# e4s2022/e4s

Hardware: AMD Instinct MI355X
Metric: 1024^2 face-swap images/sec (higher is better)
Workload: dtype f32 operands as hi+lo bf16, 3 bf16 MFMAs per product, f32 accumulate (bf16x3) on the 3x3 convs whose launch fills the chip; exact f32 elsewhere; 1 GPU; E4S-core face swap at 1024^2 (2x Net3 encoder @256^2, style swap, 12 LocalMLPs, mask-guided StyleGAN2 generator K=13), BASELINE.json configs[3] shard: 8 swaps per GPU per step; per_gpu_batch=8, global_batch=8, out_size=1024, hip_graph=True, precision=as bf16x3 where the launch fills the chip (this batch), else exact fp32, parallelism=image-parallel x1

## Files before the change

e4s_amd/csrc/common.h:

```cpp
#pragma once
#include <hip/hip_runtime.h>
#include <stdint.h>
#include <atomic>
#include "e4s_hip.h"

typedef float f32x4 __attribute__((ext_vector_type(4)));
typedef float f32x16 __attribute__((ext_vector_type(16)));

#define E4S_CHECK_LAUNCH()                         \
    do {                                           \
        hipError_t e__ = hipGetLastError();        \
        if (e__ != hipSuccess) return (int)e__;    \
    } while (0)

static inline hipStream_t as_stream(void* s) { return reinterpret_cast<hipStream_t>(s); }

__device__ __forceinline__ float wave_sum(float v) {
#pragma unroll
    for (int o = 32; o > 0; o >>= 1) v += __shfl_xor(v, o, 64);
    return v;
}

template <int N, int CNT, int O>
__device__ __forceinline__ void packed_wave_sum_step(float (&v)[N], const int lane) {
// ... 26 lines not shown
               : __int_as_float(__builtin_amdgcn_mov_dpp(__float_as_int(v), 0x4E, 0xF, 0xF, true));
}

__device__ __forceinline__ void quad_transpose4(float& a0, float& a1, float& a2, float& a3, const int lane) {
    const bool odd = lane & 1, hi = lane & 2;
    const float r01 = e4s_dpp_f32(odd ? a0 : a1, 0xB1), r23 = e4s_dpp_f32(odd ? a2 : a3, 0xB1);
    if (odd) { a0 = r01; a2 = r23; } else { a1 = r01; a3 = r23; }
    const float ra = e4s_dpp_f32(hi ? a0 : a2, 0x4E), rb = e4s_dpp_f32(hi ? a1 : a3, 0x4E);
    if (hi) { a0 = ra; a1 = rb; } else { a2 = ra; a3 = rb; }
}

__device__ __forceinline__ int xcd_remap(int bid, int nblk) {
    const int q = nblk >> 3, r = nblk & 7;
    const int xcd = bid & 7, slot = bid >> 3;
    const int base = (xcd < r) ? xcd * (q + 1) : r * (q + 1) + (xcd - r) * q;
    return base + slot;
}

static inline int e4s_ensure_dyn_smem(const void* fn, int bytes, std::atomic<uint64_t>& mask) {
    int dev = 0;
    hipError_t e = hipGetDevice(&dev);
    if (e != hipSuccess) return (int)e;
    const uint64_t bit = 1ull << (dev & 63);
    if (mask.load(std::memory_order_acquire) & bit) return 0;
    e = hipFuncSetAttribute(fn, hipFuncAttributeMaxDynamicSharedMemorySize, bytes);
    if (e != hipSuccess) return (int)e;
    mask.fetch_or(bit, std::memory_order_release);
    return 0;
}

int e4s_splitk_epilogue(const e4s_conv_params& p, int ksplit, hipStream_t st);

static inline int cdiv(int64_t a, int64_t b) { return (int)((a + b - 1) / b); }
```

e4s_amd/csrc/conv_bf16x3.hip:

```cpp
#include "common.h"
#include <stdlib.h>

namespace {

typedef __bf16 bf16x8 __attribute__((ext_vector_type(8)));
typedef float f32x8 __attribute__((ext_vector_type(8)));

constexpr int KC = 32;
constexpr int ROWB = 144;
constexpr int LO = 64;
constexpr int TW = 16, HALO_W = TW + 2;
constexpr int PBM = 256, PTH = 16, PHALO = (PTH + 2) * HALO_W;
constexpr int PNTHR = 512;

template <int BN_, int WM_, int WN_, int TPS_, int KCH_ = 32>
struct PCfg {
    static constexpr int BN = BN_, WM = WM_, WN = WN_, TPS = TPS_, KCH = KCH_;
    static constexpr int TM = PBM / (WM * 32), TN = BN / (WN * 32);
    static constexpr int ROWB = KCH == 32 ? 144 : 80;
    static constexpr int LO = KCH * 2;
    static constexpr int QG = KCH / 8;
    static constexpr int KSTEPS = KCH / 16;
    static constexpr int ITEMS = PHALO * QG;
    static constexpr int A_BYTES = PHALO * ROWB;
// ... 1115 lines not shown
    static_assert(SMEM <= 160 * 1024, "LDS budget");
    static std::atomic<uint64_t> smem_set{0};
    if (int e = e4s_ensure_dyn_smem(reinterpret_cast<const void*>(kern), SMEM, smem_set)) return e;
    const int ngemm = SHUF ? 4 * p.Cout : p.Cout;
    const int ntn = ngemm / C::BN;
    const int tx_n = (p.Wa + TW - 1) / TW, per_img = ((p.Ha + PTH - 1) / PTH) * tx_n;
    int ksplit, cper;
    plain_split(p, ngemm / C::BN, ksplit, cper);
    cper *= 32 / C::KCH;
    if (ksplit > 1 && !p.splitk_ws) return (int)hipErrorInvalidValue;
    const int64_t ntiles = (int64_t)p.B * per_img * ntn * ksplit;
    if (ntiles <= 0) return 0;
    if (ntiles >= (1ll << 31)) return (int)hipErrorInvalidValue;
    const int grid = (int)(ntiles < num_cus() ? ntiles : num_cus());
    hipLaunchKernelGGL(kern, dim3((unsigned)grid), dim3(PNTHR), SMEM, st, p, ntn, tx_n, per_img, (int)ntiles, ksplit, cper);
    E4S_CHECK_LAUNCH();
    if (ksplit > 1) {
        const int ycs = p.y_cstride ? p.y_cstride : p.Cout;
        const int64_t npix = (int64_t)p.B * p.Ho * p.Wo;
        const int64_t n4 = npix * (p.Cout / 4);
        hipLaunchKernelGGL(splitk_epilogue_kernel, dim3((unsigned)((n4 + 255) / 256)), dim3(256), 0, st, p, ksplit, ycs,
                           (int64_t)p.Ho * p.Wo, n4);
        E4S_CHECK_LAUNCH();
    }
    return 0;
}

template <typename C, bool SHUF>
int launch_xf(const e4s_conv_params& p, hipStream_t st) {
    if (p.in_stats) return SHUF ? (int)hipErrorInvalidValue : launch<C, 2, false>(p, st);
    return p.in_scale ? launch<C, 1, SHUF>(p, st) : launch<C, 0, SHUF>(p, st);
}

}

int e4s_launch_region_select(const e4s_conv_params& p, const int* only_flagged, hipStream_t st) {
    return launch_region(p, only_flagged, st);
}
void e4s_region_split_policy(const e4s_conv_params& p, int& ksplit, int& cper) { region_split(p, ksplit, cper); }

extern "C" int e4s_conv_bf16x3_f32(const e4s_conv_params* pp, void* stream) {
    const e4s_conv_params& p = *pp;
    const bool up = (p.ncls == 4);
    if (p.istride == 2 || p.ntaps == 1) {
        if (p.Cin % KC || (p.Cout % BN && p.Cout != 64) || (p.ntaps != 9 && p.ntaps != 1) || p.ncls != 1 || p.ostride != 1 || p.tiles ||
            p.labels || p.in_scale || p.out_scale || p.in_stats || p.noise || p.Ho != p.Ha || p.Wo != p.Wa ||
            p.Hi >= 32767 || p.Wi >= 32767 || (p.Ha - 1) * p.istride >= p.Hi || (p.Wa - 1) * p.istride >= p.Wi ||
            p.tap_shift < 0 || p.tap_shift > 1 ||
            (p.stats_ws && (p.act != 0 || (p.Ha * p.Wa) % BM || p.stats_slots != (p.Ha * p.Wa) / BM)))
            return (int)hipErrorInvalidValue;
        return launch_gather(p, as_stream(stream));
    }
    if (p.Cin % KC || p.Cout % 32 || p.ntaps != 9 || (p.ncls != 1 && !up) || p.istride != 1 ||
        p.ostride != (up ? 2 : 1) || p.tiles || p.noise_per_channel || p.Ha != p.Hi || p.Wa != p.Wi ||
        p.Ho != p.Hi * p.ostride || p.Wo != p.Wi * p.ostride || (p.in_stats && p.in_scale))
        return (int)hipErrorInvalidValue;
    if (p.stats_ws && (p.labels || up || p.act != 0 || p.noise || p.out_scale ||
                       p.stats_slots != ((p.Ha + PTH - 1) / PTH) * ((p.Wa + TW - 1) / TW)))
        return (int)hipErrorInvalidValue;
    hipStream_t st = as_stream(stream);
    if (p.labels) {
        if (p.y_cstride || !p.in_scale || p.in_stats || p.act == 2 || p.Cout % BN || p.groups_per_batch < 1 || p.groups_per_batch > MAXR)
            return (int)hipErrorInvalidValue;
        return launch_region(p, nullptr, st);
    }
#ifdef E4S_ABLATIONS
    static const int abl = [] { const char* e = getenv("E4S_BF16X3_ABL"); return e ? atoi(e) : 0; }();
    if (abl && !up && p.Cout % 128 == 0 && !p.in_stats && !p.in_scale) {
        switch (abl) {
            case 1: return launch<CfgL, 0, false, 1>(p, st);
            case 2: return launch<CfgL, 0, false, 2>(p, st);
            case 3: return launch<CfgL, 0, false, 3>(p, st);
            case 4: return launch<CfgL, 0, false, 4>(p, st);
            case 5: return launch<CfgL, 0, false, 5>(p, st);
            default: break;
        }
    }
#endif
    if (up) {
        if ((4 * p.Cout) % 128) return (int)hipErrorInvalidValue;
        return launch_xf<CfgL, true>(p, st);
    }
// ... 5 lines not shown
    if (p.Cout % 64 == 0) return launch_xf<CfgM, false>(p, st);
    return launch_xf<CfgS, false>(p, st);
}

int e4s_splitk_epilogue(const e4s_conv_params& p, int ksplit, hipStream_t st) {
    if (!p.splitk_ws || ksplit < 2 || p.Cout % 4) return (int)hipErrorInvalidValue;
    e4s_conv_params q = p;
    q.out_scale = nullptr;
    const int ycs = p.y_cstride ? p.y_cstride : p.Cout;
    const int64_t n4 = (int64_t)p.B * p.Ho * p.Wo * (p.Cout / 4);
    hipLaunchKernelGGL(splitk_epilogue_kernel, dim3((unsigned)((n4 + 255) / 256)), dim3(256), 0, st, q, ksplit, ycs,
                       (int64_t)p.Ho * p.Wo, n4);
    E4S_CHECK_LAUNCH();
    return 0;
}

extern "C" int64_t e4s_conv_bf16x3_ws_floats(const e4s_conv_params* pp) {
    const e4s_conv_params& p = *pp;
    if (p.istride != 1 || p.ntaps != 9 || p.Cin % KC) return 0;
    if (p.labels) {
        int ksplit, cper;
        region_split(p, ksplit, cper);
        return ksplit > 1 ? (int64_t)ksplit * p.B * p.Ho * p.Wo * p.Cout : 0;
    }
    const bool up = (p.ncls == 4);
    const int ngemm = up ? 4 * p.Cout : p.Cout;
    const int bn = (up || p.Cout % 128 == 0) ? 128 : (p.Cout % 64 == 0 ? 64 : 32);
    int ksplit, cper;
    plain_split(p, ngemm / bn, ksplit, cper);
    if (ksplit <= 1) return 0;
    return (int64_t)ksplit * p.B * p.Ho * p.Wo * (p.y_cstride ? p.y_cstride : p.Cout);
}

extern "C" int e4s_split_bf16x2_f32(const float* w, void* out, int64_t rows, int cin, void* stream) {
    if (cin % 32) return (int)hipErrorInvalidValue;
    const int64_t n8 = rows * (cin / 8);
    if (n8 <= 0) return 0;
    hipLaunchKernelGGL(split_bf16x2_kernel, dim3(cdiv(n8, 256)), dim3(256), 0, as_stream(stream), w,
                       reinterpret_cast<unsigned short*>(out), n8, cin);
    E4S_CHECK_LAUNCH();
    return 0;
}
```

e4s_amd/csrc/ops.hip:

```cpp
#include "common.h"

namespace {

__device__ __forceinline__ float bias_act_one(float x, float ref, int code, float alpha, float scale) {
    float y;
    switch (code) {
        case 12: case 32: y = 0.f; break;
        case 30: y = (x > 0.f) ? x : x * alpha; break;
        case 31: y = (ref > 0.f) ? x : x * alpha; break;
        default: y = x; break;
    }
    return y * scale;
}

__global__ void fused_bias_act_v4(const f32x4* __restrict__ x, const float* __restrict__ b,
                                  const f32x4* __restrict__ ref, f32x4* __restrict__ y, int64_t n4,
                                  int step_b, int size_b, int code, float alpha, float scale) {
    const int64_t stride = (int64_t)gridDim.x * blockDim.x;
    for (int64_t i = (int64_t)blockIdx.x * blockDim.x + threadIdx.x; i < n4; i += stride) {
        f32x4 v = x[i];
        if (b) {
            const float bv = b[((i * 4) / step_b) % size_b];
            v += bv;
        }
// ... 57 lines not shown
    for (int t = threadIdx.x; t < kh * kw; t += blockDim.x) {
        const int ky = t / kw, kx = t - ky * kw;
        sk[t] = k[(kh - 1 - ky) * kw + (kw - 1 - kx)];
    }
    const int mid_y0 = oy0 * down_y - pad_y0, mid_x0 = ox0 * down_x - pad_x0;
    const int in_y0 = floordiv(mid_y0 + up_y - 1, up_y), in_x0 = floordiv(mid_x0 + up_x - 1, up_x);
    for (int t = threadIdx.x; t < tin_h * tin_w; t += blockDim.x) {
        const int ry = t / tin_w, rx = t - ry * tin_w;
        const int iy = in_y0 + ry, ix = in_x0 + rx;
        float v = 0.f;
        if (iy >= 0 && ix >= 0 && iy < in_h && ix < in_w)
            v = x[(((int64_t)mj * in_h + iy) * in_w + ix) * minor + mi];
        sx[t] = v;
    }
    __syncthreads();
    for (int t = threadIdx.x; t < TOH * TOW; t += blockDim.x) {
        const int ry = t / TOW, rx = t - ry * TOW;
        const int oy = oy0 + ry, ox = ox0 + rx;
        if (oy >= out_h || ox >= out_w) continue;
        const int my = oy * down_y - pad_y0, mx = ox * down_x - pad_x0;
        const int iy_first = floordiv(my + up_y - 1, up_y), ix_first = floordiv(mx + up_x - 1, up_x);
        float acc = 0.f;
        for (int iy = iy_first, jy = iy_first * up_y - my; jy < kh; ++iy, jy += up_y) {
            const float* row = sx + (iy - in_y0) * tin_w;
            for (int ix = ix_first, jx = ix_first * up_x - mx; jx < kw; ++ix, jx += up_x)
                acc += row[ix - in_x0] * sk[jy * kw + jx];
        }
        y[(((int64_t)mj * out_h + oy) * out_w + ox) * minor + mi] = acc;
    }
}

}

extern "C" int e4s_abi_version(void) { return 16; }
extern "C" const char* e4s_build_arch(void) { return "gfx950"; }

extern "C" int e4s_fused_bias_act_f32(const float* x, const float* b, const float* ref, float* y, int64_t n,
                                      int step_b, int size_b, int act, int grad, float alpha, float scale,
                                      void* stream) {
    if (n <= 0) return 0;
    const int code = act * 10 + grad;
    if (code == 31 && !ref) return (int)hipErrorInvalidValue;
    if (b && (step_b <= 0 || size_b <= 0)) return (int)hipErrorInvalidValue;
    const bool vec = (n % 4 == 0) && (!b || step_b % 4 == 0) &&
                     ((reinterpret_cast<uintptr_t>(x) | reinterpret_cast<uintptr_t>(y) |
                       reinterpret_cast<uintptr_t>(ref)) % 16 == 0);
    const int block = 256;
    if (vec) {
        const int64_t n4 = n / 4;
        const int grid = (int)((n4 + block - 1) / block < 8192 ? (n4 + block - 1) / block : 8192);
        hipLaunchKernelGGL(fused_bias_act_v4, dim3(grid), dim3(block), 0, as_stream(stream),
                           reinterpret_cast<const f32x4*>(x), b, reinterpret_cast<const f32x4*>(ref),
                           reinterpret_cast<f32x4*>(y), n4, step_b, size_b, code, alpha, scale);
    } else {
        const int grid = (int)((n + block - 1) / block < 8192 ? (n + block - 1) / block : 8192);
        hipLaunchKernelGGL(fused_bias_act_scalar, dim3(grid), dim3(block), 0, as_stream(stream), x, b, ref, y, n,
                           step_b, size_b, code, alpha, scale);
    }
    E4S_CHECK_LAUNCH();
    return 0;
}

extern "C" int e4s_channel_sum_f32(const float* g, float* out, int64_t n, int step_b, int size_b, void* stream) {
    if (size_b <= 0 || step_b <= 0 || n % ((int64_t)step_b * size_b)) return (int)hipErrorInvalidValue;
    hipLaunchKernelGGL(channel_sum_kernel, dim3(size_b), dim3(256), 0, as_stream(stream), g, out, n, step_b, size_b);
    E4S_CHECK_LAUNCH();
    return 0;
// ... 117 lines not shown
```

e4s_amd/encoders.py:

```python
from collections import namedtuple

import torch
from torch import nn
from torch.nn import Conv2d, InstanceNorm2d, MaxPool2d, Module, PReLU, ReLU, Sequential, Sigmoid, AdaptiveAvgPool2d

from . import kernels as K
from .packs import param_key


class Bottleneck(namedtuple("Block", ["in_channel", "depth", "stride"])):
    """helpers.py:21-22"""


def get_block(in_channel, depth, num_units, stride=2):
    return [Bottleneck(in_channel, depth, stride)] + [Bottleneck(depth, depth, 1) for _ in range(num_units - 1)]


def _pack3x3(conv):
    w = conv.weight
    key = param_key(w)
    if getattr(conv, "_e4s_pack", None) is None or conv._e4s_pack[0] != key:
        with torch.no_grad():
            conv._e4s_pack = (key, K.pack_taps(w.detach().float().contiguous()))
    return conv._e4s_pack[1]


def _conv3x3(x, conv, cout, in_stats=None, want_stats=False, **kw):
    w = _pack3x3(conv)
    if K.wino_eligible(x.shape[0], x.shape[1], x.shape[2], x.shape[3], cout, in_stats=in_stats is not None) and set(kw) <= {"bias", "slope", "act", "alpha", "gain", "se"} \
            and not (want_stats and kw.get("act", 0) != 0):
        if getattr(conv, "_e4s_wino", None) is None or conv._e4s_wino[0] != conv._e4s_pack[0]:
            conv._e4s_wino = (conv._e4s_pack[0], K.wino_weights(w))
        return K.conv_wino(x, conv._e4s_wino[1], cout, in_stats=in_stats, want_stats=want_stats, **kw)
    if K.want_bf16x3(x.shape[0], x.shape[1], x.shape[2], x.shape[3], cout):
        if getattr(conv, "_e4s_split", None) is None or conv._e4s_split[0] != conv._e4s_pack[0]:
            conv._e4s_split = (conv._e4s_pack[0], K.split_bf16x2(w))
        return K.conv_mfma(x, w, cout, w_split=conv._e4s_split[1], in_stats=in_stats, want_stats=want_stats, **kw)
    if in_stats is not None:
        x = K.instnorm_apply(x, in_stats)
    return K.conv_mfma(x, w, cout, want_stats=want_stats, **kw)


def _conv_strided(x, conv, cout, stride, ntaps, want_stats=False, se=None, **kw):
    w = _pack3x3(conv)
    b, h, wd, _ = x.shape
    covered = cout % 128 == 0 or cout == 64
    tiles = (b * (h // stride) * (wd // stride) + 255) // 256 * ((cout + 127) // 128 if covered else 0)
    if K.PRECISION != "f32" and covered and (K.PRECISION == "bf16x3" or tiles >= K.BF16X3_MIN_BLOCKS):
        if getattr(conv, "_e4s_split", None) is None or conv._e4s_split[0] != conv._e4s_pack[0]:
            conv._e4s_split = (conv._e4s_pack[0], K.split_bf16x2(w))
        return K.conv_mfma(x, w, cout, istride=stride, ntaps=ntaps, w_split=conv._e4s_split[1], want_stats=want_stats, se=se, **kw)
    return K.conv_mfma(x, w, cout, istride=stride, ntaps=ntaps, want_stats=want_stats, se=se, **kw)


class SEModule(Module):

    def __init__(self, channels, reduction):
        super().__init__()
        self.avg_pool = AdaptiveAvgPool2d(1)
        self.fc1 = Conv2d(channels, channels // reduction, kernel_size=1, padding=0, bias=False)
        self.relu = ReLU(inplace=True)
        self.fc2 = Conv2d(channels // reduction, channels, kernel_size=1, padding=0, bias=False)
        self.sigmoid = Sigmoid()

    def forward(self, x):
        return x * torch.sigmoid(self.fc2(torch.relu(self.fc1(x.mean((2, 3), keepdim=True)))))


class bottleneck_IR_SE_Ours(Module):

    def __init__(self, in_channel, depth, stride):
        super().__init__()
        self.in_channel, self.depth, self.stride = in_channel, depth, stride
        if in_channel == depth:
            self.shortcut_layer = MaxPool2d(1, stride)
        else:
            self.shortcut_layer = Sequential(Conv2d(in_channel, depth, (1, 1), stride, bias=False),
                                             InstanceNorm2d(depth))
        self.res_layer = Sequential(InstanceNorm2d(in_channel),
                                    Conv2d(in_channel, depth, (3, 3), (1, 1), 1, bias=False),
                                    PReLU(depth),
                                    Conv2d(depth, depth, (3, 3), stride, 1, bias=False),
                                    InstanceNorm2d(depth),
                                    SEModule(depth, 16))
# ... 65 lines not shown
```

e4s_amd/kernels.py:

```python
import contextlib
import ctypes
import math
import os
import threading

import torch

from . import lib
from .lib import ConvBwdParams, ConvParams, ConvWgradParams, c_p, call, fptr, ptr, stream

BM = 128
PRECISION = os.environ.get("E4S_PRECISION", "auto")
if PRECISION not in ("f32", "bf16x3", "auto"):
    raise RuntimeError(f"E4S_PRECISION must be f32, bf16x3 or auto, got {PRECISION!r}")
BF16X3_MIN_BLOCKS = int(os.environ.get("E4S_BF16X3_MIN_BLOCKS", "128"))
LRELU_GAIN = math.sqrt(2.0)


def _f32(t):
    if t.dtype != torch.float32:
        raise RuntimeError(f"expected float32 tensor, got {t.dtype}")
    return t.contiguous()


# ... 263 lines not shown
        p.tiles_cap = 0
        p.groups_per_batch = num_regions if labels is not None else 1
    if labels is not None:
        p.labels, p.Hm, p.Wm = ptr(labels), labels.shape[1], labels.shape[2]
    else:
        p.labels, p.Hm, p.Wm = None, 0, 0
    p.B, p.Ha, p.Wa = b, ha, wa
    p.Hi, p.Wi, p.Ho, p.Wo, p.Cin, p.Cout = hi, wi, ho, wo, cin, cout
    p.istride, p.ostride, p.ntaps, p.ncls = istride, ostride, ntaps, ncls
    p.in_scale, p.out_scale = fptr(in_scale), fptr(out_scale)
    if noise is not None:
        p.noise, p.noise_w = fptr(noise), fptr(noise_w)
        p.noise_bstride = ho * wo if noise.shape[0] > 1 else 0
        p.noise_per_channel = 1 if noise_per_channel else 0
    else:
        p.noise = p.noise_w = None
        p.noise_bstride = 0
        p.noise_per_channel = 0
    p.bias, p.slope = fptr(bias), fptr(slope)
    p.act, p.alpha, p.gain = act, alpha, gain
    p.in_stats = fptr(in_stats)
    p.split_hint = 1 if getattr(_split_tl, "on", False) else 0
    if w_split is not None:
        gather_ok = (istride == 2 or ntaps == 1) and cin % 32 == 0 and (cout % 128 == 0 or cout == 64) and ncls == 1 and ostride == 1 \
            and plan is None and labels is None and in_scale is None and out_scale is None and noise is None \
            and in_stats is None
        if not gather_ok and (
                not bf16x3_eligible(cin, cout, istride=istride, ostride=ostride, ntaps=ntaps, ncls=ncls,
                                    masked=labels is not None)
                or not spatial or noise_per_channel or (labels is not None and in_scale is None)
                or (in_stats is not None and (in_scale is not None or labels is not None))):
            raise RuntimeError("e4s_conv_bf16x3_f32 does not cover this contraction")
        p.w = fptr(w_split)
        if w_split16 is not None:
            if labels is None or out is not None:
                raise RuntimeError("e4s_conv_region_bf16x3_f32 is the masked-layer kernel")
            nws = lib.load().e4s_conv_region_ws_floats(ctypes.byref(p))
            if nws <= 0:
                raise RuntimeError("e4s_conv_region_bf16x3_f32 does not cover this contraction")
            skws = torch.empty(nws, device=x.device, dtype=torch.float32)
            p.splitk_ws = fptr(skws)
            global LAST_REGION_PATH
            LAST_REGION_PATH = lib.load().e4s_conv_region_path(ctypes.byref(p))
            call("e4s_conv_region_bf16x3_f32", ctypes.byref(p), ptr(w_split16), stream())
            return y
        nws = lib.load().e4s_conv_bf16x3_ws_floats(ctypes.byref(p))
        skws = torch.empty(nws, device=x.device, dtype=torch.float32) if nws else None
        p.splitk_ws = fptr(skws)
        fused = None
        if want_stats and nws == 0 and act == 0 and noise is None and out_scale is None and labels is None and ncls == 1 \
                and cout % 64 == 0 and out is None:
            if gather_ok:
                slots = (ha * wa) // 256 if (ha * wa) % 256 == 0 else 0
            else:
                slots = ((ha + 15) // 16) * ((wa + 15) // 16)
            if slots:
                fused = torch.empty(b * cout * slots * 2, device=x.device, dtype=torch.float64)
                p.stats_ws, p.stats_slots = ptr(fused), slots
        call("e4s_conv_bf16x3_f32", ctypes.byref(p), stream())
        if fused is not None:
            stats = torch.empty(b, cout, 2, device=x.device, dtype=torch.float32)
            pooled = torch.empty(b, cout, device=x.device, dtype=torch.float32)
            if se is not None:
                call("e4s_instnorm_finalize_se_f32", ptr(fused), fptr(stats), fptr(se[0]), fptr(se[1]), fptr(pooled), b, ho * wo,
                     cout, se[0].shape[0], p.stats_slots, 1e-5, stream())
            else:
                call("e4s_instnorm_finalize_f32", ptr(fused), fptr(stats), fptr(pooled), b, ho * wo, cout, p.stats_slots, 1e-5,
                     stream())
            return y, (stats, pooled)
    elif in_stats is not None:
        raise RuntimeError("fused InstanceNorm staging exists only in e4s_conv_bf16x3_f32")
    else:
        nws = lib.load().e4s_conv_mfma_ws_floats(ctypes.byref(p), 1 if spatial else 0)
        skws = torch.empty(nws, device=x.device, dtype=torch.float32) if nws else None
        p.splitk_ws = fptr(skws)
        call("e4s_conv_mfma_f32", ctypes.byref(p), 1 if spatial else 0, stream())
    if want_stats:
        stats, pooled = instnorm_stats(y, want_pooled=True)
        return y, (stats, se_gate(pooled, se[0], se[1]) if se is not None else pooled)
    return y


def bf16x3_eligible(cin, cout, *, istride=1, ostride=1, ntaps=9, ncls=1, masked=False):
    return (cin % 32 == 0 and cout % (128 if masked else 32) == 0 and istride == 1 and ntaps == 9
            and (ncls, ostride) in ((1, 1), (4, 2)))


def want_bf16x3(b, h, w, cin, cout, ncls=1, masked=False):
# ... 6 lines not shown
    tiles = b * ((h + 15) // 16) * ((w + 15) // 16) * (n // bn) * (ncls if masked else 1)
    if tiles >= BF16X3_MIN_BLOCKS:
        return True
    nchunk = cin // 32
    split = min(nchunk // 2, -(-256 // tiles)) if nchunk >= 4 else 1
    return tiles * max(split, 1) >= 64


def split_bf16x2(w, out=None):
    w = _f32(w)
    out = _into(out, tuple(w.shape), w.device)
    cin = w.shape[-1]
    call("e4s_split_bf16x2_f32", fptr(w), ptr(out), w.numel() // cin, cin, stream())
    return out


def split16_shape(w_shape):
    return (2 if w_shape[-2] % 32 == 0 else 1,) + tuple(w_shape)


def split16_bf16x2(w, out=None):
    w = _f32(w)
    out = _into(out, split16_shape(w.shape), w.device)
    cout, cin = w.shape[-2], w.shape[-1]
    rows = w.numel() // (cout * cin)
    if lib.load().e4s_split16_bytes(rows, cout, cin) != out.numel() * 4:
        raise RuntimeError("split16_bf16x2: buffer size")
    call("e4s_split16_bf16x2_f32", fptr(w), ptr(out), rows, cout, cin, stream())
    return out


REGION_1W = os.environ.get("E4S_REGION_1W", "1") != "0"
LAST_REGION_PATH = 0
WINO = os.environ.get("E4S_WINO", "1") == "1"


def wino_eligible(b, h, w, cin, cout, in_stats=False):
    if not WINO or PRECISION == "f32":
        return False
    if h % 16 or w % 16 or cin % 16 or cin < 32 or cout % 128:
        return False
    if in_stats and cin > 1024:
        return False
    if PRECISION == "bf16x3":
        return True
    tiles = b * (h // 16) * (w // 16) * (cout // 128)
    if tiles >= BF16X3_MIN_BLOCKS:
        return True
    nchunk = cin // 16
    split = min(nchunk // 2, -(-256 // tiles)) if nchunk >= 4 else 1
    return tiles * max(split, 1) >= 64


def wino_weights(w9):
    w9 = _f32(w9)
    cout, cin = w9.shape[-2], w9.shape[-1]
    if w9.numel() != 9 * cout * cin:
        raise RuntimeError("wino_weights: one set of nine taps [9, Cout, Cin]")
    n = lib.load().e4s_wino_weights_bytes(cout, cin)
    if n <= 0:
        raise RuntimeError("wino_weights: Cin must be a multiple of 16")
    out = torch.empty(n, device=w9.device, dtype=torch.uint8)
    call("e4s_wino_weights_f32", fptr(w9), ptr(out), cout, cin, stream())
    return out


# ... 934 lines not shown
```

e4s_amd/lib.py:

```python
import ctypes
import os

import torch

_HERE = os.path.dirname(os.path.abspath(__file__))
LIB_PATH = os.environ.get("E4S_LIB_PATH") or os.path.join(_HERE, "libe4s_hip.so")
ABI_VERSION = 16

c_p = ctypes.c_void_p
c_i = ctypes.c_int
c_l = ctypes.c_int64
c_f = ctypes.c_float
c_d = ctypes.c_double


STYLE_GRAD_MAX_JOBS = 32


class StyleGradJob(ctypes.Structure):
    _fields_ = [
        ("ds_raw", c_p), ("dd_d", c_p), ("d", c_p), ("s", c_p), ("wsq", c_p), ("dws", c_p), ("w3", c_p), ("wmod", c_p), ("ds_total", c_p),
        ("conv_scale", c_f), ("mod_scale", c_f), ("G", c_i), ("Cin", c_i), ("Cout", c_i), ("slot", c_i), ("masked", c_i),
    ]


class ConvParams(ctypes.Structure):
    _fields_ = [
        ("x", c_p), ("w", c_p), ("y", c_p), ("rows", c_p), ("tiles", c_p), ("meta", c_p), ("tiles_cap", c_i),
        ("B", c_i), ("Ha", c_i), ("Wa", c_i),
        ("Hi", c_i), ("Wi", c_i), ("Ho", c_i), ("Wo", c_i), ("Cin", c_i), ("Cout", c_i),
        ("istride", c_i), ("ostride", c_i), ("ntaps", c_i), ("ncls", c_i),
        ("in_scale", c_p), ("out_scale", c_p), ("groups_per_batch", c_i),
        ("labels", c_p), ("Hm", c_i), ("Wm", c_i),
        ("noise", c_p), ("noise_w", c_p), ("noise_bstride", c_l), ("noise_per_channel", c_i),
        ("bias", c_p), ("slope", c_p), ("act", c_i), ("alpha", c_f), ("gain", c_f),
        ("in_stats", c_p), ("y_cstride", c_i), ("splitk_ws", c_p), ("stats_ws", c_p), ("stats_slots", c_i), ("tap_shift", c_i),
        ("split_hint", c_i),
    ]


class ConvBwdParams(ctypes.Structure):
    _fields_ = [
        ("gz", c_p), ("wt", c_p), ("dx", c_p), ("x", c_p), ("ds", c_p), ("s", c_p), ("d", c_p), ("labels", c_p),
        ("Hm", c_i), ("Wm", c_i), ("R", c_i),
        ("B", c_i), ("Hx", c_i), ("Wx", c_i), ("Cx", c_i), ("Hy", c_i), ("Wy", c_i), ("Cy", c_i),
        ("ncls", c_i), ("ds_ws", c_p),
    ]


class ConvWgradParams(ctypes.Structure):
    _fields_ = [
        ("gz", c_p), ("x", c_p), ("dw", c_p), ("ws", c_p), ("s", c_p), ("d", c_p), ("labels", c_p),
        ("Hm", c_i), ("Wm", c_i), ("R", c_i),
        ("B", c_i), ("Hi", c_i), ("Wi", c_i), ("Cin", c_i), ("Ha", c_i), ("Wa", c_i), ("Ho", c_i), ("Wo", c_i), ("Cout", c_i),
        ("istride", c_i), ("ostride", c_i), ("py", c_i), ("px", c_i), ("ntaps", c_i), ("tap_shift", c_i),
    ]


SIGNATURES = {
    "e4s_fused_bias_act_f32": [c_p, c_p, c_p, c_p, c_l, c_i, c_i, c_i, c_i, c_f, c_f, c_p],
    "e4s_upfirdn2d_f32": [c_p, c_p, c_p] + [c_i] * 14 + [c_p],
    "e4s_channel_sum_f32": [c_p, c_p, c_l, c_i, c_i, c_p],
    "e4s_rowdot_f32": [c_p, c_l, c_p, c_p, c_p, c_i, c_i, c_i, c_i, c_f, c_p],
    "e4s_weight_sqsum_f32": [c_p, c_p, c_i, c_i, c_i, c_p],
    "e4s_pack_taps_f32": [c_p, c_p, c_i, c_i, c_i, c_p],
    "e4s_polyphase_weights_f32": [c_p, c_p, c_p, c_i, c_i, c_p],
    "e4s_polyphase_fold_f32": [c_p, c_p, c_p, c_i, c_i, c_p],
    "e4s_rgb_weights_f32": [c_p, c_p, c_p, c_i, c_i, c_f, c_p],
    "e4s_mask_labels": [c_p, c_p, c_p, c_i, c_i, c_i, c_i, c_p],
    "e4s_region_plan": [c_p] + [c_i] * 8 + [c_p, c_p, c_p, c_p, c_i, c_i, c_p],
    "e4s_conv_mfma_f32": [ctypes.POINTER(ConvParams), c_i, c_p],
    "e4s_upconv_mfma_f32": [ctypes.POINTER(ConvParams), c_p, c_p],
    "e4s_conv_bf16x3_f32": [ctypes.POINTER(ConvParams), c_p],
    "e4s_conv_bf16x3_ws_floats": [ctypes.POINTER(ConvParams)],
    "e4s_conv_mfma_ws_floats": [ctypes.POINTER(ConvParams), c_i],
    "e4s_split_bf16x2_f32": [c_p, c_p, c_l, c_i, c_p],
    "e4s_conv_region_bf16x3_f32": [ctypes.POINTER(ConvParams), c_p, c_p],
    "e4s_conv_region_ws_floats": [ctypes.POINTER(ConvParams)],
    "e4s_conv_region_path": [ctypes.POINTER(ConvParams)],
    "e4s_split16_bytes": [ctypes.c_int64, c_i, c_i],
    "e4s_split16_bf16x2_f32": [c_p, c_p, c_l, c_i, c_i, c_p],
    "e4s_upconv_blocks_per_cu": [],
    "e4s_instnorm_ws_doubles": [c_i, c_i, c_i],
    "e4s_conv_bwd_mfma_f32": [ctypes.POINTER(ConvBwdParams), c_p],
    "e4s_pack_taps_bwd_f32": [c_p, c_p, c_i, c_i, c_i, c_p],
    "e4s_demod_grad_f32": [c_p, c_p, c_p, c_p, c_l, c_p, c_f, c_f, c_p, c_i, c_i, c_i, c_p, c_p, c_i, c_i, c_i, c_i, c_p],
    "e4s_torgb_bwd_w_f32": [c_p, c_p, c_p, c_i, c_i, c_i, c_p, c_p, c_i, c_i, c_i, c_i, c_p],
    "e4s_conv_bwd_ws_floats": [ctypes.POINTER(ConvBwdParams)],
    "e4s_seg_reduce_nsplit": [c_i, c_i, c_i, c_i],
    "e4s_grouped_linear_t_f32": [c_p, c_p, c_p, c_p, c_i, c_i, c_i, c_i, c_f, c_p, c_p, c_p, c_f, c_p],
    "e4s_grouped_linear_t_ws_floats": [c_i, c_i, c_i, c_i],
    "e4s_reduce_parts_f32": [c_p, c_p, c_i, c_l, c_f, c_p],
    "e4s_reduce_parts_ws_floats": [c_i, c_l],
    "e4s_grouped_outer_f32": [c_p, c_p, c_p, c_i, c_i, c_i, c_i, c_f, c_p],
    "e4s_style_grad_multi_f32": [c_p, c_i, c_p, c_i, c_i, c_i, c_i, c_p],
    "e4s_swap_styles_f32": [c_p, c_p, c_p, c_i, c_i, c_i, ctypes.c_uint, c_i, c_i, c_i, c_p],
    "e4s_batch_sum_f32": [c_p, c_p, c_i, c_l, c_p],
    "e4s_adam_step_f32": [c_p, c_p, c_p, c_p, c_l, c_d, c_d, c_d, c_d, c_d, c_i, c_p],
    "e4s_subpixel_weights_f32": [c_p, c_p, c_i, c_i, c_p],
    "e4s_upconv_bf16x3_f32": [c_p, c_p, c_p],
    "e4s_colsum_f32": [c_p, c_p, c_p, c_l, c_i, c_p],
    "e4s_colsum_ws_floats": [c_l, c_i],
    "e4s_scale_dot_f32": [c_p, c_p, c_p, c_p, c_p, c_i, c_l, c_i, c_p],
    "e4s_scale_dot_ws_floats": [c_i, c_l, c_i],
    "e4s_mask_to_u8": [c_p, c_p, c_i, c_i, c_i, c_i, c_i, c_p],
    "e4s_erode_u8": [c_p, c_p, c_i, c_i, c_i, c_i, c_i, c_p],
    "e4s_gaussian_blur_u8": [c_p, c_p, c_i, c_i, c_i, c_i, ctypes.POINTER(c_i), c_p],
# ... 151 lines not shown
```

e4s_amd/packs.py:

```python

_GENERATION = 0

PACK_ATTRS = (
    "_e4s_pack", "_e4s_wino", "_e4s_split", "_e4s_wt", "_e4s_wt_fwd",
    "_e4s_t", "_e4s_stats", "_e4s_head", "_e4s_small", "_e4s_fold",
    "_e4s_dpacks",
    "_mlp_pack",
    "_pack",
)


def invalidate_packs():
    global _GENERATION
    _GENERATION += 1


def invalidate_module_packs(modules):
    for m in modules:
        d = vars(m)
        for name in PACK_ATTRS:
            if d.get(name) is not None:
                d[name] = None


def modules_owning(root, params):
    ids = {id(p) for p in params}
    return [m for m in root.modules() if any(id(p) in ids for p in m.parameters())]


def param_key(*tensors):
    return (_GENERATION,) + tuple((t.data_ptr(), t._version) for t in tensors)
```

include/e4s_hip.h:

```cpp
#ifndef E4S_HIP_H
#define E4S_HIP_H
#include <stdint.h>

#ifdef __cplusplus
extern "C" {
#endif

int e4s_abi_version(void);
const char* e4s_build_arch(void);


int e4s_fused_bias_act_f32(const float* x, const float* b, const float* ref, float* y, int64_t n,
                           int step_b, int size_b, int act, int grad, float alpha, float scale,
                           void* stream);

int e4s_upfirdn2d_f32(const float* x, const float* k, float* y, int major, int in_h, int in_w, int minor,
                      int kh, int kw, int up_x, int up_y, int down_x, int down_y,
                      int pad_x0, int pad_x1, int pad_y0, int pad_y1, void* stream);

int e4s_channel_sum_f32(const float* g, float* out, int64_t n, int step_b, int size_b, void* stream);


int e4s_rowdot_f32(const float* in, int64_t in_stride, const float* M, const float* bias, float* out,
                   int G, int O, int K, int mode, float scale, void* stream);
// ... 27 lines not shown
    const float* x;
    const float* w;
    float* y;
    const int* rows;
    const int* tiles;
    const int* meta;
    int tiles_cap;
    int B, Ha, Wa;
    int Hi, Wi, Ho, Wo, Cin, Cout;
    int istride;
    int ostride;
    int ntaps;
    int ncls;
    const float* in_scale;
    const float* out_scale;
    int groups_per_batch;
    const uint8_t* labels;
    int Hm, Wm;
    const float* noise;
    const float* noise_w;
    int64_t noise_bstride;
    int noise_per_channel;
    const float* bias;
    const float* slope;
    int act;
    float alpha, gain;
    const float* in_stats;
    int y_cstride;
    float* splitk_ws;
    double* stats_ws;
    int stats_slots;
    int tap_shift;
    int split_hint;
} e4s_conv_params;

int e4s_conv_mfma_f32(const e4s_conv_params* p, int spatial, void* stream);
int64_t e4s_conv_mfma_ws_floats(const e4s_conv_params* p, int spatial);

int e4s_upconv_mfma_f32(const e4s_conv_params* p, const float* k4, void* stream);
int e4s_upconv_blocks_per_cu(void);

int e4s_conv_bf16x3_f32(const e4s_conv_params* p, void* stream);
int64_t e4s_conv_bf16x3_ws_floats(const e4s_conv_params* p);
int e4s_split_bf16x2_f32(const float* w, void* out, int64_t rows, int cin, void* stream);

int e4s_conv_region_bf16x3_f32(const e4s_conv_params* p, const void* w16, void* stream);
int64_t e4s_conv_region_ws_floats(const e4s_conv_params* p);
int e4s_conv_region_path(const e4s_conv_params* p);
int e4s_split16_bf16x2_f32(const float* w, void* out, int64_t rows, int cout, int cin, void* stream);
int64_t e4s_split16_bytes(int64_t rows, int cout, int cin);

typedef struct {
    const float* gz;
    const float* wt;
    float* dx;
    const float* x;
    float* ds;
    const float* s;
    const float* d;
    const uint8_t* labels;
    int Hm, Wm, R;
    int B, Hx, Wx, Cx, Hy, Wy, Cy;
    int ncls;
    float* ds_ws;
} e4s_conv_bwd_params;

int e4s_conv_bwd_mfma_f32(const e4s_conv_bwd_params* p, void* stream);
int64_t e4s_conv_bwd_ws_floats(const e4s_conv_bwd_params* p);
typedef struct {
    const float* gz;
    const float* x;
    float* dw;
    float* ws;
    const float* s;
    const float* d;
    const uint8_t* labels;
// ... 211 lines not shown
```

Measured before the change: 479.1 images/s.

## Add dedicated stride-2 3x3 bf16x3 conv kernel with parity-plane LDS halo tiles

Adds a new kernel for stride-2 3x3 convolutions that stages a 2D input halo tile into LDS, split into four parity planes, as hi/lo bf16. All nine taps then reuse that tile instead of going through the generic gather path. It double-buffers the K chunks, overlaps the next chunk's global loads with the MFMAs, and fuses bias, activation and the optional channel-stats epilogue. It uses a new 16-channel weight split (w16) and plumbs path and stats-slot queries through the Python side. The costs are a new pre-split weight pack per conv and a differently shaped stats-slot layout.

```diff
diff --git a/e4s_amd/csrc/common.h b/e4s_amd/csrc/common.h
--- a/e4s_amd/csrc/common.h
+++ b/e4s_amd/csrc/common.h
@@ -82,3 +82,7 @@
 int e4s_splitk_epilogue(const e4s_conv_params& p, int ksplit, hipStream_t st);
 
 static inline int cdiv(int64_t a, int64_t b) { return (int)((a + b - 1) / b); }
+
+bool e4s_conv_s2_takes(const e4s_conv_params& p);
+int e4s_conv_s2_slots(const e4s_conv_params& p);
+int e4s_launch_conv_s2(const e4s_conv_params& p, hipStream_t st);
diff --git a/e4s_amd/csrc/conv_bf16x3.hip b/e4s_amd/csrc/conv_bf16x3.hip
--- a/e4s_amd/csrc/conv_bf16x3.hip
+++ b/e4s_amd/csrc/conv_bf16x3.hip
@@ -1171,6 +1171,13 @@
     return p.in_scale ? launch<C, 1, SHUF>(p, st) : launch<C, 0, SHUF>(p, st);
 }
 
+bool gather_args_ok(const e4s_conv_params& p) {
+    return !(p.Cin % 16 || (p.Cout % BN && p.Cout != 64) || (p.ntaps != 9 && p.ntaps != 1) || p.ncls != 1 || p.ostride != 1 || p.tiles ||
+             p.labels || p.in_scale || p.out_scale || p.in_stats || p.noise || p.Ho != p.Ha || p.Wo != p.Wa ||
+             p.Hi >= 32767 || p.Wi >= 32767 || (p.Ha - 1) * p.istride >= p.Hi || (p.Wa - 1) * p.istride >= p.Wi ||
+             p.tap_shift < 0 || p.tap_shift > 1);
+}
+
 }
 
 int e4s_launch_region_select(const e4s_conv_params& p, const int* only_flagged, hipStream_t st) {
@@ -1182,11 +1189,9 @@
     const e4s_conv_params& p = *pp;
     const bool up = (p.ncls == 4);
     if (p.istride == 2 || p.ntaps == 1) {
-        if (p.Cin % KC || (p.Cout % BN && p.Cout != 64) || (p.ntaps != 9 && p.ntaps != 1) || p.ncls != 1 || p.ostride != 1 || p.tiles ||
-            p.labels || p.in_scale || p.out_scale || p.in_stats || p.noise || p.Ho != p.Ha || p.Wo != p.Wa ||
-            p.Hi >= 32767 || p.Wi >= 32767 || (p.Ha - 1) * p.istride >= p.Hi || (p.Wa - 1) * p.istride >= p.Wi ||
-            p.tap_shift < 0 || p.tap_shift > 1 ||
-            (p.stats_ws && (p.act != 0 || (p.Ha * p.Wa) % BM || p.stats_slots != (p.Ha * p.Wa) / BM)))
+        if (!gather_args_ok(p)) return (int)hipErrorInvalidValue;
+        if (e4s_conv_s2_takes(p)) return e4s_launch_conv_s2(p, as_stream(stream));
+        if (p.Cin % KC || (p.stats_ws && (p.act != 0 || (p.Ha * p.Wa) % BM || p.stats_slots != (p.Ha * p.Wa) / BM)))
             return (int)hipErrorInvalidValue;
         return launch_gather(p, as_stream(stream));
     }
@@ -1258,6 +1263,22 @@
     return (int64_t)ksplit * p.B * p.Ho * p.Wo * (p.y_cstride ? p.y_cstride : p.Cout);
 }
 
+extern "C" int e4s_conv_bf16x3_path(const e4s_conv_params* pp) {
+    const e4s_conv_params& p = *pp;
+    if (p.istride != 2 && p.ntaps != 1) return 0;
+    return (gather_args_ok(p) && e4s_conv_s2_takes(p)) ? 2 : 1;
+}
+
+extern "C" int e4s_conv_bf16x3_stats_slots(const e4s_conv_params* pp) {
+    const e4s_conv_params& p = *pp;
+    if (e4s_conv_bf16x3_ws_floats(pp) != 0) return 0;
+    switch (e4s_conv_bf16x3_path(pp)) {
+        case 2: return e4s_conv_s2_slots(p);
+        case 1: return (p.Ha * p.Wa) % BM ? 0 : (p.Ha * p.Wa) / BM;
+        default: return ((p.Ha + PTH - 1) / PTH) * ((p.Wa + TW - 1) / TW);
+    }
+}
+
 extern "C" int e4s_split_bf16x2_f32(const float* w, void* out, int64_t rows, int cin, void* stream) {
     if (cin % 32) return (int)hipErrorInvalidValue;
     const int64_t n8 = rows * (cin / 8);
diff --git a/e4s_amd/csrc/conv_s2.hip b/e4s_amd/csrc/conv_s2.hip
--- /dev/null
+++ b/e4s_amd/csrc/conv_s2.hip
@@ -0,0 +1,273 @@
+#include "common.h"
+#include <stdlib.h>
+
+namespace {
+
+typedef __bf16 bf16x8 __attribute__((ext_vector_type(8)));
+typedef float f32x8 __attribute__((ext_vector_type(8)));
+
+constexpr int NTHR = 512, BM = 256, BN = 128, TH = 8, TW = 32, KC = 16, ROWB = 64;
+constexpr int WN = 2, WM = 4, TM = 2, TN = 2;
+constexpr int HALO_W = 2 * TW + 1;
+constexpr int PW0 = TW + 1, PW1 = TW, PH0 = TH + 1, PH1 = TH;
+constexpr int BASE00 = 0, BASE01 = PH0 * PW0, BASE10 = BASE01 + PH0 * PW1, BASE11 = BASE10 + PH1 * PW0, NROW = BASE11 + PH1 * PW1;
+constexpr int A_BYTES = NROW * ROWB;
+constexpr int NITEM = NROW * 2, NIT = (NITEM + NTHR - 1) / NTHR;
+constexpr int SMEM = 2 * A_BYTES + BM * 4;
+static_assert(WM * TM == TH && TW == 32 && NROW == (2 * TH + 1) * HALO_W && NIT <= 8, "tile shape");
+static_assert(A_BYTES % 64 == 0 && WM * BN * 16 <= A_BYTES && SMEM <= 160 * 1024, "LDS budget");
+
+__host__ __device__ constexpr int plane_base(int a, int b) { return a ? (b ? BASE11 : BASE10) : (b ? BASE01 : BASE00); }
+__host__ __device__ constexpr int plane_w(int b) { return b ? PW1 : PW0; }
+__device__ __forceinline__ int swz(int row, int g) { return row * ROWB + ((g ^ ((row >> 2) & 3) ^ (row & 2)) << 4); }
+
+__device__ __forceinline__ f32x8 load8(const float* src) {
+    const f32x4 lo4 = *reinterpret_cast<const f32x4*>(src);
+    const f32x4 hi4 = *reinterpret_cast<const f32x4*>(src + 4);
+    return f32x8{lo4[0], lo4[1], lo4[2], lo4[3], hi4[0], hi4[1], hi4[2], hi4[3]};
+}
+
+struct BFrag { bf16x8 h[TN], l[TN]; };
+struct AFrag { bf16x8 h, l; };
+
+__global__ __launch_bounds__(NTHR) void conv_s2_bf16x3_kernel(const e4s_conv_params p, const unsigned char* __restrict__ wf,
+                                                              const int ntn, const int tx_n, const int per_img) {
+    extern __shared__ __attribute__((aligned(16))) unsigned char smem[];
+    unsigned char* sA = smem;
+    int* s_out = reinterpret_cast<int*>(smem + 2 * A_BYTES);
+
+    const int tid = threadIdx.x;
+    const int lane = tid & 63, wave = __builtin_amdgcn_readfirstlane(tid >> 6);
+    const int li = lane & 31, kh = lane >> 5;
+    const int wm = wave / WN, wn = wave % WN;
+    const int logical = xcd_remap(blockIdx.x, gridDim.x);
+    const int mt = logical / ntn, nt = logical - mt * ntn;
+    const int n0 = nt * BN;
+    const int tb = mt / per_img;
+    const int rem = mt - tb * per_img;
+    const int tyb = rem / tx_n, txb = rem - tyb * tx_n;
+
+    if (tid < BM) {
+        const int oy = tyb * TH + tid / TW, ox = txb * TW + tid % TW;
+        s_out[tid] = (oy < p.Ho && ox < p.Wo) ? (tb * p.Ho + oy) * p.Wo + ox : -1;
+    }
+    const int ncols = min(BN, p.Cout - n0);
+    const bool cols_live = wn * TN * 32 < ncols;
+    const int nchunk = p.Cin / KC;
+
+    int g_off[NIT], l_off[NIT];
+#pragma unroll
+    for (int j = 0; j < NIT; ++j) {
+        const int it = tid + NTHR * j;
+        const int row = it >> 1, q = it & 1;
+        const int a = row >= BASE10, b = a ? row >= BASE11 : row >= BASE01;
+        const int r = row - plane_base(a, b), pw = plane_w(b);
+        const int u = r / pw, v = r - u * pw;
+        const int iy = 2 * TH * tyb - 1 + 2 * u + a, ix = 2 * TW * txb - 1 + 2 * v + b;
+        const bool valid = it < NITEM;
+        const bool ok = valid && (unsigned)iy < (unsigned)p.Hi && (unsigned)ix < (unsigned)p.Wi;
+        g_off[j] = ok ? (iy * p.Wi + ix) * p.Cin + q * 8 : -1;
+        l_off[j] = valid ? swz(row, q) : -1;
+    }
+    const float* xb = p.x + (size_t)tb * p.Hi * p.Wi * p.Cin;
+    const f32x8 zero8 = {0.f, 0.f, 0.f, 0.f, 0.f, 0.f, 0.f, 0.f};
+    auto fetch_item = [&](int j, const float* xc) -> f32x8 { return load8(xc + max(g_off[j], 0)); };
+    auto store_item = [&](int j, unsigned char* buf, f32x8 v) {
+        if (l_off[j] < 0) return;
+        if (g_off[j] < 0) v = zero8;
+        const bf16x8 h = __builtin_convertvector(v, bf16x8);
+        const f32x8 res = v - __builtin_convertvector(h, f32x8);
+        const bf16x8 l = __builtin_convertvector(res, bf16x8);
+        *reinterpret_cast<bf16x8*>(buf + l_off[j]) = h;
+        *reinterpret_cast<bf16x8*>(buf + (l_off[j] ^ 32)) = l;
+    };
+
+    const int cb_n = p.Cout / 32;
+    const unsigned char* wfb = wf + ((size_t)(n0 / 32 + (cols_live ? wn * TN : 0)) * 2048 + lane * 16);
+    auto ldB = [&](BFrag& F, int tap, int chunk) {
+        const unsigned char* s = wfb + (size_t)(tap * nchunk + chunk) * cb_n * 2048;
+#pragma unroll
+        for (int tn = 0; tn < TN; ++tn) {
+            F.h[tn] = *reinterpret_cast<const bf16x8*>(s + tn * 2048);
+            F.l[tn] = *reinterpret_cast<const bf16x8*>(s + tn * 2048 + 1024);
+        }
+    };
+    auto ldA = [&](AFrag& F, const unsigned char* Ab, int tap, int tm) {
+        const int ky = tap / 3, kx = tap - 3 * ky;
+        const int row = plane_base(ky & 1, kx & 1) + (wm * TM + tm + (ky >> 1)) * plane_w(kx & 1) + (kx >> 1) + li;
+        const int off = swz(row, kh);
+        F.h = *reinterpret_cast<const bf16x8*>(Ab + off);
+        F.l = *reinterpret_cast<const bf16x8*>(Ab + (off ^ 32));
+    };
+
+    f32x16 acc[TM][TN];
+#pragma unroll
+    for (int tm = 0; tm < TM; ++tm)
+#pragma unroll
+        for (int tn = 0; tn < TN; ++tn)
+#pragma unroll
+            for (int r = 0; r < 16; ++r) acc[tm][tn][r] = 0.f;
+
+    BFrag B0, B1;
+    if (cols_live) ldB(B0, 0, 0);
+    {
+        f32x8 v[NIT];
+#pragma unroll
+        for (int j = 0; j < NIT; ++j) v[j] = fetch_item(j, xb);
+#pragma unroll
+        for (int j = 0; j < NIT; ++j) store_item(j, sA, v[j]);
+    }
+    __syncthreads();
+
+    for (int chunk = 0; chunk < nchunk; ++chunk) {
+        const unsigned char* Ab = sA + (chunk & 1) * A_BYTES;
+        unsigned char* An = sA + ((chunk + 1) & 1) * A_BYTES;
+        const bool have_next = chunk + 1 < nchunk;
+        const float* xn = xb + (have_next ? (chunk + 1) * KC : 0);
+        f32x8 pa[2];
+        if (!cols_live) {
+            if (have_next) {
+#pragma unroll
+                for (int j = 0; j < NIT; ++j) store_item(j, An, fetch_item(j, xn));
+            }
+            __syncthreads();
+            continue;
+        }
+        AFrag A0, A1;
+        ldA(A0, Ab, 0, 0);
+        __builtin_amdgcn_sched_barrier(0);
+#pragma unroll
+        for (int g = 0; g < 9 * TM; ++g) {
+            const int tap = g / TM, tm = g - tap * TM;
+            AFrag& Ac = (g & 1) ? A1 : A0;
+            AFrag& Anx = (g & 1) ? A0 : A1;
+            BFrag& Bc = (tap & 1) ? B1 : B0;
+            BFrag& Bn = (tap & 1) ? B0 : B1;
+            if (g + 1 < 9 * TM) ldA(Anx, Ab, (g + 1) / TM, (g + 1) % TM);
+            if (tm == 0) {
+                ldB(Bn, tap + 1 < 9 ? tap + 1 : 0, tap + 1 < 9 ? chunk : (have_next ? chunk + 1 : 0));
+                if (tap < NIT) pa[tap & 1] = fetch_item(tap, xn);
+            }
+            if (tm == TM - 1 && tap >= 1 && tap - 1 < NIT && have_next) store_item(tap - 1, An, pa[(tap - 1) & 1]);
+#pragma unroll
+            for (int tn = 0; tn < TN; ++tn)
+                acc[tm][tn] = __builtin_amdgcn_mfma_f32_32x32x16_bf16(Ac.l, Bc.h[tn], acc[tm][tn], 0, 0, 0);
+#pragma unroll
+            for (int tn = 0; tn < TN; ++tn)
+                acc[tm][tn] = __builtin_amdgcn_mfma_f32_32x32x16_bf16(Ac.h, Bc.l[tn], acc[tm][tn], 0, 0, 0);
+#pragma unroll
+            for (int tn = 0; tn < TN; ++tn)
+                acc[tm][tn] = __builtin_amdgcn_mfma_f32_32x32x16_bf16(Ac.h, Bc.h[tn], acc[tm][tn], 0, 0, 0);
+            __builtin_amdgcn_sched_barrier(0);
+        }
+        B0 = B1;
+        __syncthreads();
+    }
+
+    float bsv[TN], slp[TN];
+#pragma unroll
+    for (int tn = 0; tn < TN; ++tn) {
+        const int col = n0 + min((wn * TN + tn) * 32 + li, ncols - 1);
+        bsv[tn] = p.bias ? p.bias[col] : 0.f;
+        slp[tn] = (p.act == 2) ? p.slope[col] : p.alpha;
+    }
+    const float gain = (p.act == 1) ? p.gain : 1.f;
+    const bool do_act = p.act != 0;
+    const bool stats = p.stats_ws != nullptr;
+    double st_s[TN], st_q[TN];
+#pragma unroll
+    for (int tn = 0; tn < TN; ++tn) st_s[tn] = st_q[tn] = 0.0;
+    const int ycs = p.y_cstride ? p.y_cstride : p.Cout;
+    const bool wide = (ycs & 3) == 0;
+#pragma unroll
+    for (int tm = 0; tm < TM; ++tm) {
+#pragma unroll
+        for (int g = 0; g < 4; ++g) {
+            float v[TN][4];
+#pragma unroll
+            for (int i = 0; i < 4; ++i) {
+                const int r = 4 * g + i;
+                const bool live = s_out[(wm * TM + tm) * 32 + i + 8 * g + 4 * kh] >= 0;
+#pragma unroll
+                for (int tn = 0; tn < TN; ++tn) {
+                    float t = acc[tm][tn][r] + bsv[tn];
+                    if (do_act) t = (t > 0.f ? t : t * slp[tn]) * gain;
+                    v[tn][i] = t;
+                    if (stats && live) { st_s[tn] += (double)t; st_q[tn] += (double)t * (double)t; }
+                }
+            }
+            if (wide) {
+#pragma unroll
+                for (int tn = 0; tn < TN; ++tn) quad_transpose4(v[tn][0], v[tn][1], v[tn][2], v[tn][3], li);
+                const int off = s_out[(wm * TM + tm) * 32 + (li & 3) + 8 * g + 4 * kh];
+                if (off >= 0 && cols_live) {
+#pragma unroll
+                    for (int tn = 0; tn < TN; ++tn)
+                        *reinterpret_cast<f32x4*>(p.y + (size_t)off * ycs + n0 + (wn * TN + tn) * 32 + (li & ~3)) =
+                            f32x4{v[tn][0], v[tn][1], v[tn][2], v[tn][3]};
+                }
+            } else {
+#pragma unroll
+                for (int i = 0; i < 4; ++i) {
+                    const int off = s_out[(wm * TM + tm) * 32 + i + 8 * g + 4 * kh];
+                    if (off < 0 || !cols_live) continue;
+#pragma unroll
+                    for (int tn = 0; tn < TN; ++tn) p.y[(size_t)off * ycs + n0 + (wn * TN + tn) * 32 + li] = v[tn][i];
+                }
+            }
+        }
+    }
+    if (stats) {
+        double* s_st = reinterpret_cast<double*>(sA);
+#pragma unroll
+        for (int tn = 0; tn < TN; ++tn) {
+            st_s[tn] += __shfl_xor(st_s[tn], 32, 64);
+            st_q[tn] += __shfl_xor(st_q[tn], 32, 64);
+            if (kh == 0) {
+                const int col = (wn * TN + tn) * 32 + li;
+                s_st[(wm * BN + col) * 2] = st_s[tn];
+                s_st[(wm * BN + col) * 2 + 1] = st_q[tn];
+            }
+        }
+        __syncthreads();
+        if (tid < ncols) {
+            double a = 0.0, q = 0.0;
+#pragma unroll
+            for (int j = 0; j < WM; ++j) { a += s_st[(j * BN + tid) * 2]; q += s_st[(j * BN + tid) * 2 + 1]; }
+            double* slot = p.stats_ws + (((size_t)tb * p.Cout + n0 + tid) * p.stats_slots + rem) * 2;
+            slot[0] = a;
+            slot[1] = q;
+        }
+    }
+}
+
+bool s2_enabled() {
+    static const bool on = [] { const char* e = getenv("E4S_CONV_S2"); return !e || atoi(e) != 0; }();
+    return on;
+}
+
+}
+
+int e4s_conv_s2_slots(const e4s_conv_params& p) { return cdiv(p.Ha, TH) * cdiv(p.Wa, TW); }
+
+bool e4s_conv_s2_takes(const e4s_conv_params& p) {
+    return s2_enabled() && p.w16 && p.istride == 2 && p.ntaps == 9 && p.tap_shift == 0 && p.Hi % 2 == 0 && p.Wi % 2 == 0 &&
+           p.Ha * 2 == p.Hi && p.Wa * 2 == p.Wi && p.Cin >= KC && p.Cin % KC == 0 && (p.Cout % BN == 0 || p.Cout == 64) &&
+           p.Ha * p.Wa >= 32 && (int64_t)p.Hi * p.Wi * p.Cin < (1ll << 31);
+}
+
+int e4s_launch_conv_s2(const e4s_conv_params& p, hipStream_t st) {
+    if (p.stats_ws && (p.act != 0 || p.stats_slots != e4s_conv_s2_slots(p))) return (int)hipErrorInvalidValue;
+    auto kern = conv_s2_bf16x3_kernel;
+    static std::atomic<uint64_t> smem_set{0};
+    if (int e = e4s_ensure_dyn_smem(reinterpret_cast<const void*>(kern), SMEM, smem_set)) return e;
+    const int ntn = (p.Cout + BN - 1) / BN;
+    const int tx_n = cdiv(p.Wa, TW), per_img = cdiv(p.Ha, TH) * tx_n;
+    const int64_t blocks = (int64_t)p.B * per_img * ntn;
+    if (blocks <= 0) return 0;
+    if (blocks >= (1ll << 31) || (int64_t)p.B * p.Ha * p.Wa >= (1ll << 31)) return (int)hipErrorInvalidValue;
+    const unsigned char* wf = reinterpret_cast<const unsigned char*>(p.w16) + (size_t)9 * p.Cout * p.Cin * 4;
+    hipLaunchKernelGGL(kern, dim3((unsigned)blocks), dim3(NTHR), SMEM, st, p, wf, ntn, tx_n, per_img);
+    E4S_CHECK_LAUNCH();
+    return 0;
+}
diff --git a/e4s_amd/csrc/ops.hip b/e4s_amd/csrc/ops.hip
--- a/e4s_amd/csrc/ops.hip
+++ b/e4s_amd/csrc/ops.hip
@@ -113,7 +113,7 @@
 
 }
 
-extern "C" int e4s_abi_version(void) { return 16; }
+extern "C" int e4s_abi_version(void) { return 17; }
 extern "C" const char* e4s_build_arch(void) { return "gfx950"; }
 
 extern "C" int e4s_fused_bias_act_f32(const float* x, const float* b, const float* ref, float* y, int64_t n,
diff --git a/e4s_amd/encoders.py b/e4s_amd/encoders.py
--- a/e4s_amd/encoders.py
+++ b/e4s_amd/encoders.py
@@ -49,7 +49,12 @@
     if K.PRECISION != "f32" and covered and (K.PRECISION == "bf16x3" or tiles >= K.BF16X3_MIN_BLOCKS):
         if getattr(conv, "_e4s_split", None) is None or conv._e4s_split[0] != conv._e4s_pack[0]:
             conv._e4s_split = (conv._e4s_pack[0], K.split_bf16x2(w))
-        return K.conv_mfma(x, w, cout, istride=stride, ntaps=ntaps, w_split=conv._e4s_split[1], want_stats=want_stats, se=se, **kw)
+        w16 = None
+        if stride == 2 and ntaps == 9 and K.CONV_S2:
+            if getattr(conv, "_e4s_split16", None) is None or conv._e4s_split16[0] != conv._e4s_pack[0]:
+                conv._e4s_split16 = (conv._e4s_pack[0], K.split16_bf16x2(w))
+            w16 = conv._e4s_split16[1]
+        return K.conv_mfma(x, w, cout, istride=stride, ntaps=ntaps, w_split=conv._e4s_split[1], w_split16=w16, want_stats=want_stats, se=se, **kw)
     return K.conv_mfma(x, w, cout, istride=stride, ntaps=ntaps, want_stats=want_stats, se=se, **kw)
 
 
diff --git a/e4s_amd/kernels.py b/e4s_amd/kernels.py
--- a/e4s_amd/kernels.py
+++ b/e4s_amd/kernels.py
@@ -319,7 +319,12 @@
                 or (in_stats is not None and (in_scale is not None or labels is not None))):
             raise RuntimeError("e4s_conv_bf16x3_f32 does not cover this contraction")
         p.w = fptr(w_split)
-        if w_split16 is not None:
+        s2_route = gather_ok and istride == 2 and ntaps == 9
+        if s2_route:
+            global LAST_S2_PATH
+            p.w16 = ptr(w_split16) if (w_split16 is not None and CONV_S2) else None
+            LAST_S2_PATH = lib.load().e4s_conv_bf16x3_path(ctypes.byref(p))
+        elif w_split16 is not None:
             if labels is None or out is not None:
                 raise RuntimeError("e4s_conv_region_bf16x3_f32 is the masked-layer kernel")
             nws = lib.load().e4s_conv_region_ws_floats(ctypes.byref(p))
@@ -337,10 +342,7 @@
         fused = None
         if want_stats and nws == 0 and act == 0 and noise is None and out_scale is None and labels is None and ncls == 1 \
                 and cout % 64 == 0 and out is None:
-            if gather_ok:
-                slots = (ha * wa) // 256 if (ha * wa) % 256 == 0 else 0
-            else:
-                slots = ((ha + 15) // 16) * ((wa + 15) // 16)
+            slots = lib.load().e4s_conv_bf16x3_stats_slots(ctypes.byref(p))
             if slots:
                 fused = torch.empty(b * cout * slots * 2, device=x.device, dtype=torch.float64)
                 p.stats_ws, p.stats_slots = ptr(fused), slots
@@ -413,6 +415,8 @@
 
 REGION_1W = os.environ.get("E4S_REGION_1W", "1") != "0"
 LAST_REGION_PATH = 0
+CONV_S2 = os.environ.get("E4S_CONV_S2", "1") != "0"
+LAST_S2_PATH = 0
 WINO = os.environ.get("E4S_WINO", "1") == "1"
 
 
diff --git a/e4s_amd/lib.py b/e4s_amd/lib.py
--- a/e4s_amd/lib.py
+++ b/e4s_amd/lib.py
@@ -5,7 +5,7 @@
 
 _HERE = os.path.dirname(os.path.abspath(__file__))
 LIB_PATH = os.environ.get("E4S_LIB_PATH") or os.path.join(_HERE, "libe4s_hip.so")
-ABI_VERSION = 16
+ABI_VERSION = 17
 
 c_p = ctypes.c_void_p
 c_i = ctypes.c_int
@@ -35,7 +35,7 @@
         ("noise", c_p), ("noise_w", c_p), ("noise_bstride", c_l), ("noise_per_channel", c_i),
         ("bias", c_p), ("slope", c_p), ("act", c_i), ("alpha", c_f), ("gain", c_f),
         ("in_stats", c_p), ("y_cstride", c_i), ("splitk_ws", c_p), ("stats_ws", c_p), ("stats_slots", c_i), ("tap_shift", c_i),
-        ("split_hint", c_i),
+        ("split_hint", c_i), ("w16", c_p),
     ]
 
 
@@ -73,6 +73,8 @@
     "e4s_upconv_mfma_f32": [ctypes.POINTER(ConvParams), c_p, c_p],
     "e4s_conv_bf16x3_f32": [ctypes.POINTER(ConvParams), c_p],
     "e4s_conv_bf16x3_ws_floats": [ctypes.POINTER(ConvParams)],
+    "e4s_conv_bf16x3_path": [ctypes.POINTER(ConvParams)],
+    "e4s_conv_bf16x3_stats_slots": [ctypes.POINTER(ConvParams)],
     "e4s_conv_mfma_ws_floats": [ctypes.POINTER(ConvParams), c_i],
     "e4s_split_bf16x2_f32": [c_p, c_p, c_l, c_i, c_p],
     "e4s_conv_region_bf16x3_f32": [ctypes.POINTER(ConvParams), c_p, c_p],
diff --git a/e4s_amd/packs.py b/e4s_amd/packs.py
--- a/e4s_amd/packs.py
+++ b/e4s_amd/packs.py
@@ -2,7 +2,7 @@
 _GENERATION = 0
 
 PACK_ATTRS = (
-    "_e4s_pack", "_e4s_wino", "_e4s_split", "_e4s_wt", "_e4s_wt_fwd",
+    "_e4s_pack", "_e4s_wino", "_e4s_split", "_e4s_split16", "_e4s_wt", "_e4s_wt_fwd",
     "_e4s_t", "_e4s_stats", "_e4s_head", "_e4s_small", "_e4s_fold",
     "_e4s_dpacks",
     "_mlp_pack",
diff --git a/include/e4s_hip.h b/include/e4s_hip.h
--- a/include/e4s_hip.h
+++ b/include/e4s_hip.h
@@ -83,6 +83,7 @@
     int stats_slots;
     int tap_shift;
     int split_hint;
+    const void* w16;
 } e4s_conv_params;
 
 int e4s_conv_mfma_f32(const e4s_conv_params* p, int spatial, void* stream);
@@ -93,6 +94,8 @@
 
 int e4s_conv_bf16x3_f32(const e4s_conv_params* p, void* stream);
 int64_t e4s_conv_bf16x3_ws_floats(const e4s_conv_params* p);
+int e4s_conv_bf16x3_path(const e4s_conv_params* p);
+int e4s_conv_bf16x3_stats_slots(const e4s_conv_params* p);
 int e4s_split_bf16x2_f32(const float* w, void* out, int64_t rows, int cin, void* stream);
 
 int e4s_conv_region_bf16x3_f32(const e4s_conv_params* p, const void* w16, void* stream);
```

New measurement: 482.2 images/s, median of 6. Within noise of the previous version (+0.6%).
